# 2Retr0/GodotGaussianSplatting

Hardware: NVIDIA H100
Metric: Msplats/s (higher is better)
Workload: dtype f32

## Files before the change

### godotgaussiansplatting_b200/csrc/compositor.cu

```cuda
#include <stdlib.h>
#include <string.h>

#include "common.cuh"

namespace gsr {

namespace {

constexpr int CHUNK = 256;
constexpr int THREADS = 128;
constexpr float MIN_ALPHA = 1.0f / 255.0f;

struct F2 { float lo, hi; };
__device__ __forceinline__ F2 pk(float lo, float hi) { F2 r; r.lo = lo; r.hi = hi; return r; }
__device__ __forceinline__ void upk(F2 v, float &lo, float &hi) { lo = v.lo; hi = v.hi; }
__device__ __forceinline__ F2 fma2(F2 a, F2 b, F2 c) { return pk(__fmaf_rn(a.lo, b.lo, c.lo), __fmaf_rn(a.hi, b.hi, c.hi)); }
__device__ __forceinline__ F2 mul2(F2 a, F2 b) { return pk(__fmul_rn(a.lo, b.lo), __fmul_rn(a.hi, b.hi)); }
__device__ __forceinline__ F2 add2(F2 a, F2 b) { return pk(__fadd_rn(a.lo, b.lo), __fadd_rn(a.hi, b.hi)); }
__device__ __forceinline__ F2 sub2(F2 a, F2 b) { return pk(__fsub_rn(a.lo, b.lo), __fsub_rn(a.hi, b.hi)); }
__device__ __forceinline__ F2 mul_add2_unfused(F2 a, F2 b, F2 c) { return add2(mul2(a, b), c); }
__device__ __forceinline__ F2 bc(float x) { return pk(x, x); }

struct Staged {
    float4 a;
    float4 b;
    float c;
    float d;
};

__device__ __forceinline__ Staged null_splat() {
    Staged s;
    s.a = make_float4(0.f, 0.f, 0.f, 0.f);
    s.b = make_float4(0.f, 0.f, 0.f, 0.f);
    s.c = 0.f;
    s.d = 0.f;
    return s;
}

template <bool DEPTH>
__device__ __forceinline__ Staged gather(const float4 *__restrict__ records, const uint32_t *__restrict__ values, uint32_t idx, float4 vz) {
    const uint32_t v = __ldg(values + idx);
    const float4 *r = records + (uint64_t)v * 3u;
    const float4 r0 = __ldg(r + 0), r1 = __ldg(r + 1), r2 = __ldg(r + 2);
    Staged s;
    s.a = make_float4(r0.x, r0.y, -0.5f * r1.x, -0.5f * r1.z);
    s.b = make_float4(-r1.y, r2.w, r2.x, r2.y);
    s.c = r2.z;
    s.d = DEPTH ? -(((vz.x * r0.z + vz.y * r0.w) + vz.z * r1.w) + vz.w * 1.0f) : 0.f;
    return s;
}

#ifndef GSR_COMP_GROUP
#define GSR_COMP_GROUP 4
#endif
constexpr int GU = GSR_COMP_GROUP;
static_assert(CHUNK % GU == 0, "a chunk is a whole number of groups");

#ifndef GSR_CPU_EMU
__device__ __forceinline__ unsigned long long globaltimer_ns() { unsigned long long t; asm volatile("mov.u64 %0, %globaltimer;" : "=l"(t)); return t; }
__device__ __forceinline__ uint32_t smid() { uint32_t r; asm volatile("mov.u32 %0, %smid;" : "=r"(r)); return r; }
#else
inline unsigned long long globaltimer_ns() { return 0ull; }
inline uint32_t smid() { return 0u; }
#endif

struct BlendK {
    F2 L2E2, MAGIC2, ONE2, C6, C5, C4, C3, C2, C1;
};
__device__ __forceinline__ BlendK make_blend_k() {
    BlendK k;
    k.L2E2 = bc(0x1.715476p+0f); k.MAGIC2 = bc(12582912.0f); k.ONE2 = bc(1.0f);
    k.C6 = bc(0x1.446c7ep-13f); k.C5 = bc(0x1.5f48c8p-10f); k.C4 = bc(0x1.3b29d8p-7f); k.C3 = bc(0x1.c6aeccp-5f);
    k.C2 = bc(0x1.ebfbe0p-3f); k.C1 = bc(0x1.62e430p-1f);
    return k;
}

template <bool CONTRACT>
__device__ __forceinline__ void phase_a(const float4 A[GU], const float4 B[GU], F2 npx2, float fpy, const BlendK &K, F2 al2[GU], F2 om2[GU]) {
    float oy[GU];
    F2 ox2[GU], pw2[GU], tm2[GU], e2[GU];
#pragma unroll
    for (int u = 0; u < GU; ++u) { ox2[u] = add2(bc(A[u].x), npx2); oy[u] = A[u].y - fpy; }
#pragma unroll
    for (int u = 0; u < GU; ++u) pw2[u] = mul2(bc(A[u].z), ox2[u]);
#pragma unroll
    for (int u = 0; u < GU; ++u) {
        const float czoy = A[u].w * oy[u];
        if (CONTRACT) pw2[u] = fma2(bc(czoy), bc(oy[u]), mul2(pw2[u], ox2[u]));
        else pw2[u] = mul_add2_unfused(pw2[u], ox2[u], bc(__fmul_rn(czoy, oy[u])));
    }
#pragma unroll
    for (int u = 0; u < GU; ++u) e2[u] = mul2(bc(B[u].x), ox2[u]);
#pragma unroll
    for (int u = 0; u < GU; ++u) pw2[u] = CONTRACT ? fma2(e2[u], bc(oy[u]), pw2[u]) : mul_add2_unfused(e2[u], bc(oy[u]), pw2[u]);
#pragma unroll
    for (int u = 0; u < GU; ++u) pw2[u] = mul2(pw2[u], K.L2E2);
#pragma unroll
    for (int u = 0; u < GU; ++u) {
        float tl, th;
        upk(pw2[u], tl, th);
        tl = g_min(g_max(tl, -127.0f), 128.0f);
        th = g_min(g_max(th, -127.0f), 128.0f);
        pw2[u] = pk(tl, th);
    }
#pragma unroll
    for (int u = 0; u < GU; ++u) tm2[u] = add2(pw2[u], K.MAGIC2);
#pragma unroll
    for (int u = 0; u < GU; ++u) al2[u] = sub2(tm2[u], K.MAGIC2);
#pragma unroll
    for (int u = 0; u < GU; ++u) pw2[u] = sub2(pw2[u], al2[u]);
#pragma unroll
    for (int u = 0; u < GU; ++u) e2[u] = fma2(K.C6, pw2[u], K.C5);
#pragma unroll
    for (int u = 0; u < GU; ++u) e2[u] = fma2(e2[u], pw2[u], K.C4);
#pragma unroll
    for (int u = 0; u < GU; ++u) e2[u] = fma2(e2[u], pw2[u], K.C3);
#pragma unroll
    for (int u = 0; u < GU; ++u) e2[u] = fma2(e2[u], pw2[u], K.C2);
#pragma unroll
    for (int u = 0; u < GU; ++u) e2[u] = fma2(e2[u], pw2[u], K.C1);
#pragma unroll
    for (int u = 0; u < GU; ++u) e2[u] = fma2(e2[u], pw2[u], K.ONE2);
#pragma unroll
    for (int u = 0; u < GU; ++u) {
        float ml, mh;
        upk(tm2[u], ml, mh);
        tm2[u] = pk(__uint_as_float((__float_as_uint(ml) << 23) + 0x3F800000u), __uint_as_float((__float_as_uint(mh) << 23) + 0x3F800000u));
    }
#pragma unroll
    for (int u = 0; u < GU; ++u) e2[u] = mul2(e2[u], tm2[u]);
#pragma unroll
    for (int u = 0; u < GU; ++u) al2[u] = mul2(bc(B[u].y), e2[u]);
#pragma unroll
    for (int u = 0; u < GU; ++u) om2[u] = sub2(K.ONE2, al2[u]);
}

template <bool CONTRACT, bool DEPTH>
__device__ __forceinline__ void phase_b(const float4 B[GU], const float *s_c, const float *s_d, int j, const F2 al2[GU], const F2 om2[GU], F2 &cr2,
                                        F2 &cg2, F2 &cb2, float &t0, float &t1, bool &alive_mid, float z0, float z1, bool &o0, bool &o1, F2 &dd2) {
#pragma unroll
    for (int u = 0; u < GU; ++u) {
        const float cbl = s_c[j + u];
        float dj = 0.f;
        bool a0, a1;
        if constexpr (DEPTH) {
            dj = s_d[j + u];
            if (u == GU / 2) alive_mid = (t0 > MIN_ALPHA && o0) || (t1 > MIN_ALPHA && o1);
            a0 = t0 > MIN_ALPHA && o0; a1 = t1 > MIN_ALPHA && o1;
            const bool v0 = dj < z0, v1 = dj < z1;
            o0 = a0 ? v0 : o0; o1 = a1 ? v1 : o1;
            a0 = a0 && v0; a1 = a1 && v1;
        } else {
            if (u == GU / 2) alive_mid = (t0 > MIN_ALPHA) || (t1 > MIN_ALPHA);
            a0 = t0 > MIN_ALPHA; a1 = t1 > MIN_ALPHA;
        }
        float al, ah, pl, ph;
        upk(al2[u], al, ah);
        const F2 t2 = pk(t0, t1);
        upk(mul2(t2, om2[u]), pl, ph);
        const F2 m2 = pk(a0 ? al : 0.0f, a1 ? ah : 0.0f);
        if (CONTRACT) {
            cr2 = fma2(mul2(bc(B[u].z), m2), t2, cr2);
            cg2 = fma2(mul2(bc(B[u].w), m2), t2, cg2);
            cb2 = fma2(mul2(bc(cbl), m2), t2, cb2);
            if constexpr (DEPTH) dd2 = fma2(mul2(bc(dj), m2), t2, dd2);
        } else {
            cr2 = mul_add2_unfused(mul2(bc(B[u].z), m2), t2, cr2);
            cg2 = mul_add2_unfused(mul2(bc(B[u].w), m2), t2, cg2);
            cb2 = mul_add2_unfused(mul2(bc(cbl), m2), t2, cb2);
            if constexpr (DEPTH) dd2 = mul_add2_unfused(mul2(bc(dj), m2), t2, dd2);
        }
        t0 = a0 ? pl : t0;
        t1 = a1 ? ph : t1;
    }
}

#ifndef GSR_COMP_MIN_BLOCKS
#define GSR_COMP_MIN_BLOCKS 3
#endif

template <bool CONTRACT, bool DEPTH = false>
__global__ void __launch_bounds__(THREADS, GSR_COMP_MIN_BLOCKS) composite_kernel(const __grid_constant__ CompositeArgs p) {
    __shared__ float4 s_a[CHUNK];
    __shared__ float4 s_b[CHUNK];
    __shared__ float s_c[CHUNK];
    __shared__ float s_d[DEPTH ? CHUNK : 1];
    __shared__ uint32_t s_vote[THREADS / 32];
    __shared__ uint32_t s_tile;

    const uint32_t tid = threadIdx.x, lane = tid & 31u, warp = tid >> 5;
    {
        const uint32_t limit = p.frame->comp_cta_limit;
        if (limit && blockIdx.x >= limit) return;
    }
    const BlendK K = make_blend_k();
    const float4 vz = DEPTH ? make_float4(p.view_z[0], p.view_z[1], p.view_z[2], p.view_z[3]) : make_float4(0.f, 0.f, 0.f, 0.f);
    uint32_t staged = 0;
    unsigned long long t_start = 0;

    for (;;) {
        if (tid == 0) {
            const uint32_t ticket = atomicAdd(&p.frame->comp_head, 1u);
            s_tile = ticket < (uint32_t)p.num_tiles ? (p.order ? p.order[ticket] : ticket) : 0xFFFFFFFFu;
            if (p.trace) t_start = globaltimer_ns();
        }
        __syncthreads();
        const uint32_t local_tile = s_tile;
        if (local_tile == 0xFFFFFFFFu) break;
        const uint32_t tile_id = (uint32_t)p.tile_begin + (local_tile / (uint32_t)p.tiles_x) * (uint32_t)(p.row_step * p.tiles_x) + local_tile % (uint32_t)p.tiles_x;

        const uint32_t tx = tile_id % (uint32_t)p.tiles_x, ty = tile_id / (uint32_t)p.tiles_x;
        const int px0 = (int)(tx * TILE + 2u * (tid & 7u)), py = (int)(ty * TILE + (tid >> 3));
        const F2 npx2 = pk(-(float)px0, -(float)(px0 + 1));
        const float fpy = (float)py;

        const uint2 bounds = p.bounds[tile_id];
        const int32_t diff = (int32_t)(bounds.y - bounds.x);
        const int num_splats = diff > 0 ? diff : 0;
        const int num_iterations = (int)ceilf((float)num_splats / (float)CHUNK);

        F2 cr2 = pk(0.f, 0.f), cg2 = cr2, cb2 = cr2;
        float t0 = 1.0f, t1 = 1.0f;
        bool o0 = true, o1 = true;
        F2 dd2 = pk(0.f, 0.f);
        float z0 = __uint_as_float(0x7f800000u), z1 = z0;
        if (DEPTH && p.scene_depth && py < p.height) {
            const float *zrow = p.scene_depth + (uint64_t)py * (uint64_t)p.width;
            if (px0 < p.width) z0 = zrow[px0];
            if (px0 + 1 < p.width) z1 = zrow[px0 + 1];
        }

        Staged n0 = null_splat(), n1 = null_splat();
        if (num_iterations > 0) {
            if ((int)tid < num_splats) n0 = gather<DEPTH>(p.records, p.values, bounds.x + tid, vz);
            if ((int)tid + THREADS < num_splats) n1 = gather<DEPTH>(p.records, p.values, bounds.x + tid + THREADS, vz);
        }

        int consumed = 0;
        for (int i = 0; i < num_iterations; ++i) {
            const int sort_offset = CHUNK * i;
            const int chunk = (num_splats - sort_offset) < CHUNK ? (num_splats - sort_offset) : CHUNK;
            staged += (uint32_t)chunk;
            consumed = i + 1;
            s_a[tid] = n0.a; s_b[tid] = n0.b; s_c[tid] = n0.c;
            s_a[tid + THREADS] = n1.a; s_b[tid + THREADS] = n1.b; s_c[tid + THREADS] = n1.c;
            if constexpr (DEPTH) { s_d[tid] = n0.d; s_d[tid + THREADS] = n1.d; }
            __syncthreads();
            n0 = null_splat(); n1 = null_splat();
            if (i + 1 < num_iterations) {
                const int nb = sort_offset + CHUNK;
                if (nb + (int)tid < num_splats) n0 = gather<DEPTH>(p.records, p.values, bounds.x + (uint32_t)nb + tid, vz);
                if (nb + (int)tid + THREADS < num_splats) n1 = gather<DEPTH>(p.records, p.values, bounds.x + (uint32_t)nb + tid + THREADS, vz);
            }

            const int chunkg = (chunk + GU - 1) & ~(GU - 1);
            float4 A[GU], B[GU];
#pragma unroll
            for (int u = 0; u < GU; ++u) { A[u] = s_a[u]; B[u] = s_b[u]; }
            bool go;
            if constexpr (DEPTH) go = __any_sync(0xffffffffu, (t0 > MIN_ALPHA && o0) || (t1 > MIN_ALPHA && o1));
            else go = __any_sync(0xffffffffu, (t0 > MIN_ALPHA) || (t1 > MIN_ALPHA));
            for (int j = 0; j < chunkg && go; j += GU) {
                F2 al2[GU], om2[GU];
                phase_a<CONTRACT>(A, B, npx2, fpy, K, al2, om2);
                float4 Bc[GU];
#pragma unroll
                for (int u = 0; u < GU; ++u) Bc[u] = B[u];
                const int jn = (j + GU < CHUNK) ? j + GU : j;
#pragma unroll
                for (int u = 0; u < GU; ++u) { A[u] = s_a[jn + u]; B[u] = s_b[jn + u]; }
                bool alive_mid = true;
                phase_b<CONTRACT, DEPTH>(Bc, s_c, s_d, j, al2, om2, cr2, cg2, cb2, t0, t1, alive_mid, z0, z1, o0, o1, dd2);
                go = __any_sync(0xffffffffu, alive_mid);
            }

            uint32_t wsum;
            if constexpr (DEPTH) wsum = __reduce_add_sync(0xffffffffu, (o0 ? (uint32_t)(t0 * 255.0f) : 0u) + (o1 ? (uint32_t)(t1 * 255.0f) : 0u));
            else wsum = __reduce_add_sync(0xffffffffu, (uint32_t)(t0 * 255.0f) + (uint32_t)(t1 * 255.0f));
            if (lane == 0) s_vote[warp] = wsum;
            __syncthreads();
            uint32_t shared_t = 0;
#pragma unroll
            for (int w = 0; w < THREADS / 32; ++w) shared_t += s_vote[w];
            if (!(shared_t > 255u)) break;
        }

        float r0, r1, g0, g1, b0, b1;
        upk(cr2, r0, r1); upk(cg2, g0, g1); upk(cb2, b0, b1);
        const float hx = (float)num_splats * 5e-4f;
        const float h0 = 0.0f * (1.0f - hx) + 1.0f * hx, h1 = 0.0f * (1.0f - hx) + 0.2f * hx, h2c = 1.0f * (1.0f - hx) + 0.2f * hx;
        if (py < p.height) {
            float4 *row = p.out + (uint64_t)py * (uint64_t)p.width;
            const float k0 = 1.0f - t0, k1 = 1.0f - t1;
            const float al0 = DEPTH ? k0 : 1.0f, al1 = DEPTH ? k1 : 1.0f;
            if (px0 < p.width)
                row[px0] = make_float4(r0 + h0 * k0 * p.heatmap_factor, g0 + h1 * k0 * p.heatmap_factor, b0 + h2c * k0 * p.heatmap_factor, al0);
            if (px0 + 1 < p.width)
                row[px0 + 1] = make_float4(r1 + h0 * k1 * p.heatmap_factor, g1 + h1 * k1 * p.heatmap_factor, b1 + h2c * k1 * p.heatmap_factor, al1);
            if (DEPTH) {
                float d0, d1;
                upk(dd2, d0, d1);
                const float inf = __uint_as_float(0x7f800000u);
                float *drow = p.depth_out + (uint64_t)py * (uint64_t)p.width;
                if (px0 < p.width) drow[px0] = k0 > 0.0f ? __fdiv_rn(d0, k0) : inf;
                if (px0 + 1 < p.width) drow[px0 + 1] = k1 > 0.0f ? __fdiv_rn(d1, k1) : inf;
            }
        }
        if ((tid & 15u) == 0u && tile_id == p.target_tile_id && t0 != 1.0f) {
            const uint32_t v = p.values[bounds.x + (bounds.y - bounds.x) / 10u];
            const float4 q0 = p.records[(uint64_t)v * 3u + 0], q1 = p.records[(uint64_t)v * 3u + 1];
            *p.pick = make_float4(q0.z, q0.w, q1.w, (float)num_splats);
        }
        if (tid == 0) {
            if (p.consumed) p.consumed[local_tile] = (uint32_t)consumed | 0x80000000u;
            if (p.trace) {
                const uint32_t k = atomicAdd(p.trace_count, 1u);
                if (k < p.trace_cap) p.trace[k] = make_ulonglong4(((unsigned long long)tile_id << 32) | smid(), t_start, globaltimer_ns(),
                                                                  ((unsigned long long)(uint32_t)consumed << 32) | 1u | ((uint32_t)num_iterations << 1));
            }
        }
        __syncthreads();
    }
    if (tid == 0 && staged && p.count_staged) atomicAdd(&p.frame->staged, (unsigned long long)staged);
}

}

#ifndef GSR_CPU_EMU
int preload_composite_kernels() {
    cudaFuncAttributes fa;
    GSR_CUDA_TRY(cudaFuncGetAttributes(&fa, composite_kernel<true>));
    GSR_CUDA_TRY(cudaFuncGetAttributes(&fa, composite_kernel<false>));
    GSR_CUDA_TRY(cudaFuncGetAttributes(&fa, composite_kernel<true, true>));
    GSR_CUDA_TRY(cudaFuncGetAttributes(&fa, composite_kernel<false, true>));
    return GSR_OK;
}

int composite_max_ctas_per_sm(int *out) {
    int a = 0, b = 0, c = 0, d = 0;
    GSR_CUDA_TRY(cudaOccupancyMaxActiveBlocksPerMultiprocessor(&a, composite_kernel<true>, THREADS, 0));
    GSR_CUDA_TRY(cudaOccupancyMaxActiveBlocksPerMultiprocessor(&b, composite_kernel<false>, THREADS, 0));
    GSR_CUDA_TRY(cudaOccupancyMaxActiveBlocksPerMultiprocessor(&c, composite_kernel<true, true>, THREADS, 0));
    GSR_CUDA_TRY(cudaOccupancyMaxActiveBlocksPerMultiprocessor(&d, composite_kernel<false, true>, THREADS, 0));
    if (c < a) a = c;
    if (d < b) b = d;
    *out = a < b ? a : b;
    if (*out < 1) *out = 1;
    return GSR_OK;
}

int launch_composite(const CompositeArgs &a, cudaStream_t stream) {
    if (a.num_tiles <= 0) return GSR_OK;
    const int per_sm = a.ctas_per_sm > 0 ? a.ctas_per_sm : 1;
    const int grid = a.num_tiles < a.sm_count * per_sm ? a.num_tiles : a.sm_count * per_sm;
    if (a.depth_out) {
        if (a.contract) composite_kernel<true, true><<<grid, THREADS, 0, stream>>>(a);
        else composite_kernel<false, true><<<grid, THREADS, 0, stream>>>(a);
    } else if (a.contract) {
        composite_kernel<true><<<grid, THREADS, 0, stream>>>(a);
    } else {
        composite_kernel<false><<<grid, THREADS, 0, stream>>>(a);
    }
    GSR_CUDA_TRY(cudaGetLastError());
    return GSR_OK;
}
#endif

}
```

Before: 3400.

## Pair pixels vertically, share x terms, and skip upper clamp for bounded splats

```diff
diff --git a/godotgaussiansplatting_b200/csrc/compositor.cu b/godotgaussiansplatting_b200/csrc/compositor.cu
--- a/godotgaussiansplatting_b200/csrc/compositor.cu
+++ b/godotgaussiansplatting_b200/csrc/compositor.cu
@@ -75,32 +75,40 @@
     return k;
 }
 
-template <bool CONTRACT>
-__device__ __forceinline__ void phase_a(const float4 A[GU], const float4 B[GU], F2 npx2, float fpy, const BlendK &K, F2 al2[GU], F2 om2[GU]) {
-    float oy[GU];
-    F2 ox2[GU], pw2[GU], tm2[GU], e2[GU];
-#pragma unroll
-    for (int u = 0; u < GU; ++u) { ox2[u] = add2(bc(A[u].x), npx2); oy[u] = A[u].y - fpy; }
-#pragma unroll
-    for (int u = 0; u < GU; ++u) pw2[u] = mul2(bc(A[u].z), ox2[u]);
+__device__ __forceinline__ bool bounded_power(const Staged &s) {
+    const float LIM = 0x1p32f;
+    const bool finite = fabsf(s.a.x) <= LIM && fabsf(s.a.y) <= LIM && fabsf(s.a.z) <= LIM && fabsf(s.a.w) <= LIM && fabsf(s.b.x) <= LIM;
+    const double b = (double)s.b.x, ac4 = 4.0 * ((double)s.a.z * (double)s.a.w);
+    return finite && s.a.z <= 0.0f && s.a.w <= 0.0f && b * b <= ac4 * (1.0 - 0x1p-16);
+}
+
+template <bool CONTRACT, bool CLAMP_HI>
+__device__ __forceinline__ void phase_a(const float4 A[GU], const float4 B[GU], float npx, F2 fpy2, const BlendK &K, F2 al2[GU], F2 om2[GU]) {
+    float ox[GU], q[GU], e[GU];
+    F2 oy2[GU], pw2[GU], tm2[GU], e2[GU];
+#pragma unroll
+    for (int u = 0; u < GU; ++u) { ox[u] = __fadd_rn(A[u].x, npx); oy2[u] = sub2(bc(A[u].y), fpy2); }
+#pragma unroll
+    for (int u = 0; u < GU; ++u) q[u] = __fmul_rn(__fmul_rn(A[u].z, ox[u]), ox[u]);
 #pragma unroll
     for (int u = 0; u < GU; ++u) {
-        const float czoy = A[u].w * oy[u];
-        if (CONTRACT) pw2[u] = fma2(bc(czoy), bc(oy[u]), mul2(pw2[u], ox2[u]));
-        else pw2[u] = mul_add2_unfused(pw2[u], ox2[u], bc(__fmul_rn(czoy, oy[u])));
-    }
-#pragma unroll
-    for (int u = 0; u < GU; ++u) e2[u] = mul2(bc(B[u].x), ox2[u]);
-#pragma unroll
-    for (int u = 0; u < GU; ++u) pw2[u] = CONTRACT ? fma2(e2[u], bc(oy[u]), pw2[u]) : mul_add2_unfused(e2[u], bc(oy[u]), pw2[u]);
+        const F2 czoy2 = mul2(bc(A[u].w), oy2[u]);
+        if (CONTRACT) pw2[u] = fma2(czoy2, oy2[u], bc(q[u]));
+        else pw2[u] = add2(bc(q[u]), mul2(czoy2, oy2[u]));
+    }
+#pragma unroll
+    for (int u = 0; u < GU; ++u) e[u] = __fmul_rn(B[u].x, ox[u]);
+#pragma unroll
+    for (int u = 0; u < GU; ++u) pw2[u] = CONTRACT ? fma2(bc(e[u]), oy2[u], pw2[u]) : mul_add2_unfused(bc(e[u]), oy2[u], pw2[u]);
 #pragma unroll
     for (int u = 0; u < GU; ++u) pw2[u] = mul2(pw2[u], K.L2E2);
 #pragma unroll
     for (int u = 0; u < GU; ++u) {
         float tl, th;
         upk(pw2[u], tl, th);
-        tl = g_min(g_max(tl, -127.0f), 128.0f);
-        th = g_min(g_max(th, -127.0f), 128.0f);
+        tl = g_max(tl, -127.0f);
+        th = g_max(th, -127.0f);
+        if (CLAMP_HI) { tl = g_min(tl, 128.0f); th = g_min(th, 128.0f); }
         pw2[u] = pk(tl, th);
     }
 #pragma unroll
@@ -175,17 +183,44 @@
     }
 }
 
+template <bool CONTRACT, bool DEPTH, bool CLAMP_HI>
+__device__ __forceinline__ void blend_chunk(const float4 *s_a, const float4 *s_b, const float *s_c, const float *s_d, int chunk, float npx, F2 fpy2,
+                                            const BlendK &K, F2 &cr2, F2 &cg2, F2 &cb2, float &t0, float &t1, float z0, float z1, bool &o0, bool &o1,
+                                            F2 &dd2) {
+    const int chunkg = (chunk + GU - 1) & ~(GU - 1);
+    float4 A[GU], B[GU];
+#pragma unroll
+    for (int u = 0; u < GU; ++u) { A[u] = s_a[u]; B[u] = s_b[u]; }
+    bool go;
+    if constexpr (DEPTH) go = __any_sync(0xffffffffu, (t0 > MIN_ALPHA && o0) || (t1 > MIN_ALPHA && o1));
+    else go = __any_sync(0xffffffffu, (t0 > MIN_ALPHA) || (t1 > MIN_ALPHA));
+#pragma unroll 2
+    for (int j = 0; j < chunkg && go; j += GU) {
+        F2 al2[GU], om2[GU];
+        phase_a<CONTRACT, CLAMP_HI>(A, B, npx, fpy2, K, al2, om2);
+        float4 Bc[GU];
+#pragma unroll
+        for (int u = 0; u < GU; ++u) Bc[u] = B[u];
+#pragma unroll
+        for (int u = 0; u < GU; ++u) { A[u] = s_a[j + GU + u]; B[u] = s_b[j + GU + u]; }
+        bool alive_mid = true;
+        phase_b<CONTRACT, DEPTH>(Bc, s_c, s_d, j, al2, om2, cr2, cg2, cb2, t0, t1, alive_mid, z0, z1, o0, o1, dd2);
+        go = __any_sync(0xffffffffu, alive_mid);
+    }
+}
+
 #ifndef GSR_COMP_MIN_BLOCKS
 #define GSR_COMP_MIN_BLOCKS 3
 #endif
 
 template <bool CONTRACT, bool DEPTH = false>
 __global__ void __launch_bounds__(THREADS, GSR_COMP_MIN_BLOCKS) composite_kernel(const __grid_constant__ CompositeArgs p) {
-    __shared__ float4 s_a[CHUNK];
-    __shared__ float4 s_b[CHUNK];
+    __shared__ float4 s_a[CHUNK + GU];
+    __shared__ float4 s_b[CHUNK + GU];
     __shared__ float s_c[CHUNK];
     __shared__ float s_d[DEPTH ? CHUNK : 1];
     __shared__ uint32_t s_vote[THREADS / 32];
+    __shared__ uint32_t s_wide[THREADS / 32];
     __shared__ uint32_t s_tile;
 
     const uint32_t tid = threadIdx.x, lane = tid & 31u, warp = tid >> 5;
@@ -193,6 +228,7 @@
         const uint32_t limit = p.frame->comp_cta_limit;
         if (limit && blockIdx.x >= limit) return;
     }
+    if (tid < (uint32_t)GU) { const Staged z = null_splat(); s_a[CHUNK + tid] = z.a; s_b[CHUNK + tid] = z.b; }
     const BlendK K = make_blend_k();
     const float4 vz = DEPTH ? make_float4(p.view_z[0], p.view_z[1], p.view_z[2], p.view_z[3]) : make_float4(0.f, 0.f, 0.f, 0.f);
     uint32_t staged = 0;
@@ -210,9 +246,9 @@
         const uint32_t tile_id = (uint32_t)p.tile_begin + (local_tile / (uint32_t)p.tiles_x) * (uint32_t)(p.row_step * p.tiles_x) + local_tile % (uint32_t)p.tiles_x;
 
         const uint32_t tx = tile_id % (uint32_t)p.tiles_x, ty = tile_id / (uint32_t)p.tiles_x;
-        const int px0 = (int)(tx * TILE + 2u * (tid & 7u)), py = (int)(ty * TILE + (tid >> 3));
-        const F2 npx2 = pk(-(float)px0, -(float)(px0 + 1));
-        const float fpy = (float)py;
+        const int px = (int)(tx * TILE + (tid & 15u)), py0 = (int)(ty * TILE + 2u * (tid >> 4));
+        const float npx = -(float)px;
+        const F2 fpy2 = pk((float)py0, (float)(py0 + 1));
 
         const uint2 bounds = p.bounds[tile_id];
         const int32_t diff = (int32_t)(bounds.y - bounds.x);
@@ -224,10 +260,10 @@
         bool o0 = true, o1 = true;
         F2 dd2 = pk(0.f, 0.f);
         float z0 = __uint_as_float(0x7f800000u), z1 = z0;
-        if (DEPTH && p.scene_depth && py < p.height) {
-            const float *zrow = p.scene_depth + (uint64_t)py * (uint64_t)p.width;
-            if (px0 < p.width) z0 = zrow[px0];
-            if (px0 + 1 < p.width) z1 = zrow[px0 + 1];
+        if (DEPTH && p.scene_depth && px < p.width) {
+            const float *zcol = p.scene_depth + (uint64_t)py0 * (uint64_t)p.width + (uint64_t)px;
+            if (py0 < p.height) z0 = zcol[0];
+            if (py0 + 1 < p.height) z1 = zcol[p.width];
         }
 
         Staged n0 = null_splat(), n1 = null_splat();
@@ -245,7 +281,14 @@
             s_a[tid] = n0.a; s_b[tid] = n0.b; s_c[tid] = n0.c;
             s_a[tid + THREADS] = n1.a; s_b[tid + THREADS] = n1.b; s_c[tid + THREADS] = n1.c;
             if constexpr (DEPTH) { s_d[tid] = n0.d; s_d[tid + THREADS] = n1.d; }
+            {
+                const bool wide = __any_sync(0xffffffffu, !(bounded_power(n0) && bounded_power(n1)));
+                if (lane == 0) s_wide[warp] = wide ? 1u : 0u;
+            }
             __syncthreads();
+            uint32_t any_wide = 0;
+#pragma unroll
+            for (int w = 0; w < THREADS / 32; ++w) any_wide |= s_wide[w];
             n0 = null_splat(); n1 = null_splat();
             if (i + 1 < num_iterations) {
                 const int nb = sort_offset + CHUNK;
@@ -253,26 +296,8 @@
                 if (nb + (int)tid + THREADS < num_splats) n1 = gather<DEPTH>(p.records, p.values, bounds.x + (uint32_t)nb + tid + THREADS, vz);
             }
 
-            const int chunkg = (chunk + GU - 1) & ~(GU - 1);
-            float4 A[GU], B[GU];
-#pragma unroll
-            for (int u = 0; u < GU; ++u) { A[u] = s_a[u]; B[u] = s_b[u]; }
-            bool go;
-            if constexpr (DEPTH) go = __any_sync(0xffffffffu, (t0 > MIN_ALPHA && o0) || (t1 > MIN_ALPHA && o1));
-            else go = __any_sync(0xffffffffu, (t0 > MIN_ALPHA) || (t1 > MIN_ALPHA));
-            for (int j = 0; j < chunkg && go; j += GU) {
-                F2 al2[GU], om2[GU];
-                phase_a<CONTRACT>(A, B, npx2, fpy, K, al2, om2);
-                float4 Bc[GU];
-#pragma unroll
-                for (int u = 0; u < GU; ++u) Bc[u] = B[u];
-                const int jn = (j + GU < CHUNK) ? j + GU : j;
-#pragma unroll
-                for (int u = 0; u < GU; ++u) { A[u] = s_a[jn + u]; B[u] = s_b[jn + u]; }
-                bool alive_mid = true;
-                phase_b<CONTRACT, DEPTH>(Bc, s_c, s_d, j, al2, om2, cr2, cg2, cb2, t0, t1, alive_mid, z0, z1, o0, o1, dd2);
-                go = __any_sync(0xffffffffu, alive_mid);
-            }
+            if (any_wide) blend_chunk<CONTRACT, DEPTH, true>(s_a, s_b, s_c, s_d, chunk, npx, fpy2, K, cr2, cg2, cb2, t0, t1, z0, z1, o0, o1, dd2);
+            else blend_chunk<CONTRACT, DEPTH, false>(s_a, s_b, s_c, s_d, chunk, npx, fpy2, K, cr2, cg2, cb2, t0, t1, z0, z1, o0, o1, dd2);
 
             uint32_t wsum;
             if constexpr (DEPTH) wsum = __reduce_add_sync(0xffffffffu, (o0 ? (uint32_t)(t0 * 255.0f) : 0u) + (o1 ? (uint32_t)(t1 * 255.0f) : 0u));
@@ -289,21 +314,20 @@
         upk(cr2, r0, r1); upk(cg2, g0, g1); upk(cb2, b0, b1);
         const float hx = (float)num_splats * 5e-4f;
         const float h0 = 0.0f * (1.0f - hx) + 1.0f * hx, h1 = 0.0f * (1.0f - hx) + 0.2f * hx, h2c = 1.0f * (1.0f - hx) + 0.2f * hx;
-        if (py < p.height) {
-            float4 *row = p.out + (uint64_t)py * (uint64_t)p.width;
+        if (px < p.width) {
+            const uint64_t o = (uint64_t)py0 * (uint64_t)p.width + (uint64_t)px;
             const float k0 = 1.0f - t0, k1 = 1.0f - t1;
             const float al0 = DEPTH ? k0 : 1.0f, al1 = DEPTH ? k1 : 1.0f;
-            if (px0 < p.width)
-                row[px0] = make_float4(r0 + h0 * k0 * p.heatmap_factor, g0 + h1 * k0 * p.heatmap_factor, b0 + h2c * k0 * p.heatmap_factor, al0);
-            if (px0 + 1 < p.width)
-                row[px0 + 1] = make_float4(r1 + h0 * k1 * p.heatmap_factor, g1 + h1 * k1 * p.heatmap_factor, b1 + h2c * k1 * p.heatmap_factor, al1);
+            if (py0 < p.height)
+                p.out[o] = make_float4(r0 + h0 * k0 * p.heatmap_factor, g0 + h1 * k0 * p.heatmap_factor, b0 + h2c * k0 * p.heatmap_factor, al0);
+            if (py0 + 1 < p.height)
+                p.out[o + (uint64_t)p.width] = make_float4(r1 + h0 * k1 * p.heatmap_factor, g1 + h1 * k1 * p.heatmap_factor, b1 + h2c * k1 * p.heatmap_factor, al1);
             if (DEPTH) {
                 float d0, d1;
                 upk(dd2, d0, d1);
                 const float inf = __uint_as_float(0x7f800000u);
-                float *drow = p.depth_out + (uint64_t)py * (uint64_t)p.width;
-                if (px0 < p.width) drow[px0] = k0 > 0.0f ? __fdiv_rn(d0, k0) : inf;
-                if (px0 + 1 < p.width) drow[px0 + 1] = k1 > 0.0f ? __fdiv_rn(d1, k1) : inf;
+                if (py0 < p.height) p.depth_out[o] = k0 > 0.0f ? __fdiv_rn(d0, k0) : inf;
+                if (py0 + 1 < p.height) p.depth_out[o + (uint64_t)p.width] = k1 > 0.0f ? __fdiv_rn(d1, k1) : inf;
             }
         }
         if ((tid & 15u) == 0u && tile_id == p.target_tile_id && t0 != 1.0f) {
diff --git a/ubench/compositor_isa.py b/ubench/compositor_isa.py
--- /dev/null
+++ b/ubench/compositor_isa.py
@@ -0,0 +1,88 @@
+import ctypes as C
+import os
+import subprocess
+import sys
+
+import numpy as np
+
+sys.path.insert(0, os.path.dirname(os.path.dirname(os.path.abspath(__file__))))
+import bench
+from godotgaussiansplatting_b200 import _lib
+from tests.gsr_direct import Ctx
+
+OTHER = os.path.abspath(sys.argv[1])
+F = int(sys.argv[2]) if len(sys.argv) > 2 else 120
+ROUNDS = int(sys.argv[3]) if len(sys.argv) > 3 else 4
+wl = dict(bench.WORKLOADS[sys.argv[4] if len(sys.argv) > 4 else "c3"])
+n, w, h = wl["n"], wl["w"], wl["h"]
+
+try:
+    gpu = subprocess.run(["nvidia-smi", "-i", "0", "--query-gpu=name,power.limit,clocks.max.sm", "--format=csv,noheader"],
+                         capture_output=True, text=True, timeout=30).stdout.strip()
+except (OSError, subprocess.SubprocessError):
+    gpu = "unknown"
+print(f"GPU: {gpu}; workload {wl['desc']}; {F} frames per library per round, {ROUNDS} rounds", flush=True)
+
+
+def context(path):
+    _lib.LIB_PATH, _lib._lib = path, None
+    c = Ctx(n, w, h)
+    for lo, blk in bench.raw_chunks(wl):
+        c.upload_ply_raw(blk, first=lo)
+    return c
+
+
+CTX = {"other": context(OTHER), "tree": context(os.path.join(os.path.dirname(_lib.__file__), "libgsr.so"))}
+FRAMES = bench.frame_params(wl, F + 10)
+
+
+def history(c, k):
+    buf = (_lib.GsrFrameRecord * k)()
+    got = C.c_uint32(0)
+    _lib.check(c.L.gsr_get_frame_history(c.h, k, buf, C.byref(got)), "gsr_get_frame_history")
+    return np.array([[buf[i].stage_ms[j] for j in range(5)] for i in range(got.value)]), np.array([buf[i].staged for i in range(got.value)])
+
+
+def run(c):
+    for i in range(10):
+        c.render_async(*FRAMES[i])
+    c.sync()
+    for i in range(10, 10 + F):
+        c.render_async(*FRAMES[i])
+    c.sync()
+    return history(c, F)
+
+
+def frame(c, i):
+    img = np.zeros((h, w, 4), dtype=np.float32)
+    c.render_async(*FRAMES[i], host_ptr=img.ctypes.data)
+    c.sync()
+    return img
+
+
+COLS = {"compositor": 3, "frame": 4}
+stages = {k: [] for k in CTX}
+staged = {k: [] for k in CTX}
+for r in range(ROUNDS):
+    for name, c in CTX.items():
+        st, cc = run(c)
+        stages[name].append(st)
+        staged[name].append(cc)
+    i = 10 + (r * 37) % F
+    same = np.array_equal(frame(CTX["other"], i).view(np.uint32), frame(CTX["tree"], i).view(np.uint32))
+    print(f"round {r}: " + "  ".join(f"{k} render {np.median(stages[k][-1][:, 3]):.4f} frame {np.median(stages[k][-1][:, 4]):.4f} ms" for k in CTX)
+          + f"  frame {i} byte-identical: {same}", flush=True)
+    assert same, f"frame {i} differs between the two libraries"
+
+print(f"median over {ROUNDS} x {F} frames; spread = min..max of the per-round medians")
+for name in CTX:
+    line = [f"  {name:5s}"]
+    for col, j in COLS.items():
+        allv = np.concatenate(stages[name])[:, j]
+        base = np.median(np.concatenate(stages["other"])[:, j])
+        rounds = [np.median(s[:, j]) for s in stages[name]]
+        line.append(f"{col} {np.median(allv):.4f} ms ({100 * (np.median(allv) / base - 1):+6.2f} %) spread {min(rounds):.4f}..{max(rounds):.4f}")
+    line.append(f"C {np.median(np.concatenate(staged[name])) / 1e6:.3f} M")
+    print("   ".join(line), flush=True)
+for c in CTX.values():
+    c.close()
diff --git a/ubench/compositor_sass.py b/ubench/compositor_sass.py
--- /dev/null
+++ b/ubench/compositor_sass.py
@@ -0,0 +1,88 @@
+import collections
+import os
+import re
+import subprocess
+import sys
+import tempfile
+
+ROOT = os.path.dirname(os.path.dirname(os.path.abspath(__file__)))
+sys.path.insert(0, ROOT)
+from godotgaussiansplatting_b200 import build as gb
+
+EVALS_PER_ITER = 4 * 2
+NAMES = {"Lb1ELb0E": "composite_kernel<true>", "Lb0ELb0E": "composite_kernel<false>",
+         "Lb1ELb1E": "composite_kernel<true, true>", "Lb0ELb1E": "composite_kernel<false, true>"}
+INSN = re.compile(r"/\*([0-9a-f]{4,})\*/\s+(.*?)\s*;")
+
+
+def compile_sass(src):
+    flags = [f for f in gb.NVCC_FLAGS if f not in ("-shared", "-Xcompiler", "-fPIC,-fvisibility=hidden", "-cudart", "shared")]
+    with tempfile.TemporaryDirectory() as tmp:
+        cubin = os.path.join(tmp, "compositor.cubin")
+        r = subprocess.run([gb.nvcc_path()] + flags + ["-I", os.path.dirname(gb.CSRC), "-I", gb.CSRC, "-I", os.path.join(ROOT, "include"),
+                                                       "-cubin", "-Xptxas", "-v", "-o", cubin, src], capture_output=True, text=True)
+        if r.returncode:
+            sys.exit(r.stdout + r.stderr)
+        sass = subprocess.run([os.path.join(os.path.dirname(gb.nvcc_path()), "cuobjdump"), "-sass", cubin], capture_output=True,
+                              text=True, check=True).stdout
+    regs, cur = collections.defaultdict(list), None
+    for line in (r.stdout + r.stderr).splitlines():
+        m = re.search(r"Compiling entry function '.*composite_kernelI(Lb[01]ELb[01]E)", line)
+        if m:
+            cur = NAMES[m.group(1)]
+        elif "Compiling entry function" in line:
+            cur = None
+        elif cur and ("registers" in line or "spill" in line):
+            regs[cur].append(re.sub(r"^ptxas info\s*:\s*", "", line.strip()))
+    return sass, {k: "; ".join(v) for k, v in regs.items()}
+
+
+def kernels(sass):
+    out, name = {}, None
+    for line in sass.splitlines():
+        m = re.search(r"Function : .*composite_kernelI(Lb[01]ELb[01]E)", line)
+        if m:
+            name = NAMES[m.group(1)]
+            out[name] = []
+        elif "Function :" in line:
+            name = None
+        elif name:
+            i = INSN.search(line)
+            if i:
+                out[name].append((int(i.group(1), 16), i.group(2)))
+    return out
+
+
+def blend_loops(insns):
+    at = {a: k for k, (a, _) in enumerate(insns)}
+    loops = []
+    for k, (addr, text) in enumerate(insns):
+        m = re.search(r"\bBRA\b.*?0x([0-9a-f]+)", text)
+        if not m or int(m.group(1), 16) >= addr or int(m.group(1), 16) not in at:
+            continue
+        body = [t for _, t in insns[at[int(m.group(1), 16)]:k + 1]]
+        if any("VOTE.ANY" in t for t in body) and any("FMNMX" in t for t in body) and not any("BAR." in t for t in body):
+            loops.append(body)
+    return loops
+
+
+def opcode(t):
+    w = t.split()
+    return (w[1] if w[0].startswith("@") else w[0]).split(".")[0]
+
+
+def main():
+    src = os.path.abspath(sys.argv[1]) if len(sys.argv) > 1 else os.path.join(gb.CSRC, "compositor.cu")
+    sass, regs = compile_sass(src)
+    print(f"{src}: blend loop of each composite_kernel instantiation ({EVALS_PER_ITER} splat-pixel evaluations per iteration)")
+    for name, insns in kernels(sass).items():
+        print(f"{name}: {len(insns)} instructions; {regs.get(name, '?')}")
+        for body in blend_loops(insns):
+            hist = collections.Counter(opcode(t) for t in body)
+            evals = EVALS_PER_ITER * hist["VOTE"]
+            print(f"    loop: {len(body)} instructions for {evals} evaluations = {len(body) / evals:.2f} per evaluation, "
+                  f"{hist['FMNMX'] / evals:.0f} clamp(s) per evaluation: " + " ".join(f"{op} {n}" for op, n in hist.most_common()))
+
+
+if __name__ == "__main__":
+    main()
```

Measured after the change: 3481 (median of 6 runs). +2.4%, better.
